# pashtari/factorizer

Measured on AMD Instinct MI355X. Metric: volumes/sec fwd+bwd, Swin Factorizer 128^3, higher is better.
Workload: dtype f32

## Files before the change

factorizer_amd/_native.py:

```python
from __future__ import annotations

import ctypes
import os
import threading

import torch

_HERE = os.path.dirname(os.path.abspath(__file__))
LIB_PATH = os.environ.get("FZ_LIB_PATH") or os.path.join(_HERE, "libfactorizer_hip.so")

FZ_OK = 0
FZ_E_UNSUPPORTED = -2
ABI_VERSION = 7
SOLVER_ID = {"mu": 0, "hals": 1, "cd": 2, "smu": 3}
STORE_F32, STORE_BF16 = 0, 1
PRODUCTS_DEFAULT, PRODUCTS_SPLIT_BF16, PRODUCTS_FP32_MFMA = 0, 1, 2
_products = threading.local()


def products() -> int:
    return getattr(_products, "value", PRODUCTS_DEFAULT)


class use_products:
# ... 150 lines not shown


class BlockPrologue(_c.Structure):
    _fields_ = [("ln_g", _vp), ("ln_b", _vp), ("ln_eps", _f), ("w", _vp), ("t", _vp), ("stats", _vp)]


class GemmDwDesc(_c.Structure):
    _fields_ = [("g", _vp), ("q", _vp), ("w", _vp), ("ln", _i), ("stats", _vp), ("ln_g", _vp), ("ln_b", _vp), ("gadd", _vp),
                ("y", _vp), ("gln", _vp), ("wpart", _vp), ("gw", _vp), ("gb", _vp), ("B", _i), ("C", _i), ("V", _i64),
                ("act_dtype", _i), ("ldgw", _i), ("ldw", _i), ("drop_m", _vp), ("drop_s", _f)]


class WgradDesc(_c.Structure):
    _fields_ = [("p", _vp), ("M", _i), ("pmul", _vp), ("pmul_kind", _i), ("q", _vp * 4), ("nsrc", _i),
                ("src_mode", _i), ("c0", _i), ("Cin", _i), ("K", _i), ("Vq", _i64), ("D", _i), ("H", _i),
                ("W", _i), ("N", _i64), ("Ho", _i), ("Wo", _i), ("stats", _vp), ("qact", _i), ("ln_g", _vp),
                ("ln_b", _vp), ("gw", _vp), ("gbias", _vp), ("accumulate", _i), ("B", _i), ("loader", _i),
                ("act_dtype", _i), ("products", _i)]


_SIGS.update({
    "fz_gcorr_supported": ([_i] * 5, _i),
    "fz_gcorr": ([_vp] * 5 + [_i] * 11 + [_f, _vp], _i),
    "fz_gcorr_wgrad_workspace_bytes": ([_i] * 10, _i64),
    "fz_gcorr_wgrad": ([_vp] * 4 + [_i] * 11 + [_vp], _i),
    "fz_gnmf_supported": ([_i, _i64, _i, _i, _i], _i),
    "fz_gnmf_workspace_bytes": ([_i64, _i, _i64, _i, _i, _i], _i64),
    "fz_gnmf_launches": ([_i, _i, _i], _i),
    "fz_gnmf_fwd": ([_vp] * 6 + [_i64, _i, _i64, _i, _i, _i, _f, _vp, _vp], _i),
    "fz_gnmf_bwd": ([_vp] * 7 + [_i64, _i, _i64, _i, _i, _i, _i, _f, _vp, _vp], _i),
    "fz_nmf_cf_supported": ([_i] * 11, _i),
    "fz_nmf_cf_fwd": ([_vp] * 4 + [_i] * 5 + [_c.POINTER(_i)] + [_i] * 5 + [_f, _i, _vp], _i),
    "fz_nmf_cf_bwd": ([_vp] * 5 + [_i] * 5 + [_c.POINTER(_i)] + [_i] * 7 + [_f, _i, _vp], _i),
    "fz_nmf_pcf_supported": ([_i] * 11, _i),
    "fz_nmf_pcf_fwd": ([_vp] * 4 + [_i] * 8 + [_c.POINTER(_i)] + [_i] * 5 + [_f, _i, _vp], _i),
    "fz_nmf_pcf_bwd": ([_vp] * 5 + [_i] * 8 + [_c.POINTER(_i)] + [_i] * 7 + [_f, _i, _vp], _i),
    "fz_nmf_pcf_bwd_prefers_separate": ([_i] * 4, _i),
    "fz_act_add": ([_vp, _vp, _i64, _i, _vp], _i),
    "fz_mlp_pre_supported": ([_i, _i, _i64, _i], _i),
    "fz_mlp_drop_supported": ([_i, _i, _i64, _i], _i),
    "fz_mlp_chain_drop": ([_c.POINTER(MlpDesc), _c.POINTER(MlpDropout), _vp], _i),
    "fz_conv3_prologue_supported": ([_i] * 4, _i),
    "fz_conv3_fwd2": ([_vp] * 4 + [_i] * 8 + [_c.POINTER(BlockPrologue), _vp], _i),
    "fz_upcat2": ([_vp, _vp, _vp, _i, _vp, _vp, _vp] + [_i] * 7 + [_c.POINTER(BlockPrologue), _vp], _i),
    "fz_gemm": ([_c.POINTER(GemmDesc), _vp], _i),
    "fz_gemm_bx_enable": ([_i], _i),
    "fz_gemm_lnbwd_partials": ([_c.POINTER(GemmDesc)], _i64),
    "fz_reduce_rows": ([_vp, _i64, _i, _vp, _vp, _vp], _i),
    "fz_adamw_step": ([_vp, _vp, _vp, _vp, _i64, _f, _f, _f, _f, _f, _i, _f, _vp], _i),
    "fz_sw_gather": ([_vp, _vp] + [_i] * 10 + [_vp], _i),
    "fz_sw_accumulate": ([_vp] * 6 + [_f] + [_i] * 10 + [_vp], _i),
    "fz_sw_finalize": ([_vp, _vp, _i, _i64, _vp], _i),
    "fz_sw_gather2": ([_vp, _vp] + [_i] * 11 + [_vp], _i),
    "fz_sw_accumulate2": ([_vp] * 6 + [_f] + [_i] * 11 + [_vp], _i),
    "fz_sw_finalize2": ([_vp, _vp, _vp, _i, _i64, _i, _vp], _i),
    "fz_mlp_supported": ([_i, _i, _i64], _i),
    "fz_mlp_partials": ([_i, _i64], _i64),
    "fz_mlp_wgrad_rows": ([_i, _i64], _i),
    "fz_gemm_dw_rows": ([_i, _i64], _i),
    "fz_gemm_dw_workspace_bytes": ([_i, _i64], _i64),
    "fz_gemm_dw": ([_c.POINTER(GemmDwDesc), _vp], _i),
    "fz_mlp_wgrad_workspace_bytes": ([_i, _i64], _i64),
    "fz_mlp_chain": ([_c.POINTER(MlpDesc), _vp], _i),
    "fz_head_bwd_rows": ([], _i),
    "fz_head_bwd_workspace_bytes": ([], _i64),
    "fz_head_bwd": ([_vp, _vp, _vp, _vp, _vp, _i, _i, _i, _i64, _i, _vp], _i),
# ... 47 lines not shown
```

factorizer_amd/csrc/nmf_cf.h:

```cpp
#pragma once
#include <cstdlib>

#include "fz_common.h"
#include "nmf_core.h"
#include "nmf_gram.h"

namespace fz {

struct CfGeom {
  int B, C, D, H, W;
  int h;
  int G0, G1, G2;
  int s0, s1, s2;
  int accumulate;
  int divisor;
  float gscale_div;
  int64_t plane;
};

struct CfWave {
  using F = float;
  int lane;
  __device__ __forceinline__ int col(int j) const {
    const int jp = j >> 2, e = j & 3;
    return (((jp * 4 + (lane >> 4)) * 8 + ((lane >> 1) & 7)) * 8) + (lane & 1) * 4 + e;
  }
  __device__ __forceinline__ float sum(float v) const { return wave_sum(v); }
  __device__ __forceinline__ void sum8(float (&v)[8]) const { wave_sum8(v, lane); }
  __device__ __forceinline__ void st_priv(float* base, int idx, float v) const { base[idx * 64 + lane] = v; }
  __device__ __forceinline__ float ld_priv(const float* base, int idx) const { return base[idx * 64 + lane]; }
  __device__ __forceinline__ void st_uni(float* base, int idx, float v) const {
    if (lane == 0) base[idx] = v;
  }
  __device__ __forceinline__ float ld_uni(const float* base, int idx) const { return base[idx]; }
  __device__ __forceinline__ float ld_uni_global(const float* p, int idx) const { return p[idx]; }
  __device__ __forceinline__ float ld_v0(const float* v0, int j, int r, int R) const { return v0[col(j) * R + r]; }
  __device__ __forceinline__ float keep_col(int, float v) const { return v; }
  __device__ __forceinline__ void fence() const { __builtin_amdgcn_fence(__ATOMIC_ACQ_REL, "wavefront"); }
  static constexpr bool kDistRows = true;
  __device__ __forceinline__ float sum8_dist(const float (&v)[8]) const { return wave_sum8_dist(v, lane); }
  __device__ __forceinline__ float grp_take(float d, int m) const {
    return __int_as_float(__builtin_amdgcn_readlane(__float_as_int(d), 8 * m));
  }
  __device__ __forceinline__ bool grp_below(int n) const { return (lane >> 3) < n; }
  __device__ __forceinline__ void st_grp(float* base, int i0, int stride, float d) const {
    if ((lane & 7) == 0) base[i0 + (lane >> 3) * stride] = d;
  }
  __device__ __forceinline__ float ld_grp_global(const float* p, int i0, int stride) const { return p[i0 + (lane >> 3) * stride]; }
  __device__ __forceinline__ float ld_grp(const float* base, int i0, int stride) const { return base[i0 + (lane >> 3) * stride]; }
  __device__ __forceinline__ float grp_sum(float d) const { return wave_group_sum(d); }
  __device__ __forceinline__ float mask_rows(float d, int mreal) const { return (lane >> 3) < mreal ? d : 0.f; }
// ... 143 lines not shown
    aload<2>(cf_at(p, o), a);
    aload<2>(cf_at(p, o2), b);
    return make_float4(a[0], a[1], b[0], b[1]);
  }
  return ld4(cf_at(p, o));
}
template <bool HALF, typename AT>
__device__ __forceinline__ void cf_st4(AT* p, unsigned o, unsigned o2, float4 v) {
  if (HALF) {
    const float a[2] = {v.x, v.y}, b[2] = {v.z, v.w};
    astore<2>(cf_at(p, o), a);
    astore<2>(cf_at(p, o2), b);
  } else {
    st4(cf_at(p, o), v);
  }
}

struct CfTileId { int b, hh, g0, g1, gq; };

template <int WPB>
__device__ __forceinline__ CfTileId cf_tile_id(const CfGeom& q, int64_t blk) {
  const unsigned ngrp = (unsigned)(q.G2 / WPB);
  unsigned t = (unsigned)blk;
  CfTileId id;
  id.gq = (int)(t % ngrp); t /= ngrp;
  id.g1 = (int)(t % (unsigned)q.G1); t /= (unsigned)q.G1;
  id.g0 = (int)(t % (unsigned)q.G0); t /= (unsigned)q.G0;
  id.hh = (int)(t % (unsigned)q.h);
  id.b = (int)(t / (unsigned)q.h);
  return id;
}

template <int WPB>
__device__ __forceinline__ void cf_tile_decode(const CfGeom& q, const CfTileId& id, int tid, int64_t& base, int64_t& V,
                                               unsigned (&off)[2], int (&lidx)[2], unsigned (&off2)[2]) {
  using TL = CfTile<WPB>;
  V = q.plane;
  base = ((int64_t)id.b * q.C + (int64_t)id.hh * 8) * V;
#pragma unroll
  for (int k = 0; k < 2; ++k) {
    const int idx = tid + k * TL::NT;
    const int row = idx / TL::CHUNKS, chunk = idx % TL::CHUNKS;
    int z0 = id.g0 * 8 + (row >> 3) - q.s0; if (z0 < 0) z0 += q.D;
    int z1 = id.g1 * 8 + (row & 7) - q.s1; if (z1 < 0) z1 += q.H;
    int z2 = id.gq * WPB * 8 + chunk * 4 - q.s2; if (z2 < 0) z2 += q.W;
    off[k] = (unsigned)((z0 * q.H + z1) * q.W + z2);
    int z2b = z2 + 2; if (z2b >= q.W) z2b -= q.W;
    off2[k] = (unsigned)((z0 * q.H + z1) * q.W + z2b);
    lidx[k] = TL::at(row, chunk);
  }
}

template <int WPB>
__device__ __forceinline__ int cf_owner_lidx(int lane, int wave, int jp) {
  return CfTile<WPB>::at((jp * 4 + (lane >> 4)) * 8 + ((lane >> 1) & 7), wave * 2 + (lane & 1));
}

template <int WPB>
__device__ __forceinline__ void cf_to_owner(float* S, const int (&lidx)[2], int own0, int own1, float (&x)[8][8]) {
  using TL = CfTile<WPB>;
#pragma unroll
  for (int s = 0; s < 4; ++s) {
#pragma unroll
    for (int c = 0; c < 2; ++c)
#pragma unroll
      for (int k = 0; k < 2; ++k)
        *reinterpret_cast<float4*>(S + c * 64 * TL::LW + lidx[k]) =
            make_float4(x[2 * s + c][k * 4 + 0], x[2 * s + c][k * 4 + 1], x[2 * s + c][k * 4 + 2], x[2 * s + c][k * 4 + 3]);
    __syncthreads();
#pragma unroll
    for (int c = 0; c < 2; ++c) {
      const float4 a0 = *reinterpret_cast<const float4*>(S + c * 64 * TL::LW + own0);
      const float4 a1 = *reinterpret_cast<const float4*>(S + c * 64 * TL::LW + own1);
      x[2 * s + c][0] = a0.x; x[2 * s + c][1] = a0.y; x[2 * s + c][2] = a0.z; x[2 * s + c][3] = a0.w;
      x[2 * s + c][4] = a1.x; x[2 * s + c][5] = a1.y; x[2 * s + c][6] = a1.z; x[2 * s + c][7] = a1.w;
    }
    __syncthreads();
  }
}


template <typename AT>
int cf_bwd_gram_launch(const AT* t, const float* v0, const AT* ga, AT* gt, const CfGeom& q, int64_t nmat, int T, int G,
// ... 4 lines not shown
```

factorizer_amd/csrc/nmf_cf.hip:

```cpp
#include "nmf_cf.h"

namespace fz {

template <int R, int SOLVER, int WPB, bool HALF, typename AT>
__device__ __forceinline__ void cf_fwd_tile_body(const AT* __restrict__ t, const float* __restrict__ u0,
                                                 const float* __restrict__ v0, AT* __restrict__ out, const CfGeom& q,
                                                 const CfTileId& id, int T, float eps, float* S) {
  using TL = CfTile<WPB>;
  const int tid = threadIdx.x, lane = tid & 63, wave = tid >> 6;
  int64_t base, V;
  unsigned off[2], off2[2];
  int lidx[2];
  cf_tile_decode<WPB>(q, id, tid, base, V, off, lidx, off2);
  const int own0 = cf_owner_lidx<WPB>(lane, wave, 0), own1 = cf_owner_lidx<WPB>(lane, wave, 1);

  float x[8][8];
#pragma unroll
  for (int dd = 0; dd < 8; ++dd)
#pragma unroll
    for (int k = 0; k < 2; ++k) {
      const float4 v = cf_ld4<HALF>(t + base + dd * V, off[k], off2[k]);
      x[dd][k * 4 + 0] = v.x; x[dd][k * 4 + 1] = v.y; x[dd][k * 4 + 2] = v.z; x[dd][k * 4 + 3] = v.w;
    }
  cf_to_owner<WPB>(S, lidx, own0, own1, x);

  CfWave w{lane};
  float u[8][R], v[8][R];
  nmf_forward_wave<8, 8, R, SOLVER>(w, u0, v0, x, u, v, 8, T, eps);

  const float dv = (float)q.divisor;
  const bool dv_pow2 = cf_pow2(dv);
  asm volatile("" : "+s"(base));
  float4 old[8][2];
  if (q.accumulate) {
#pragma unroll
    for (int dd = 0; dd < 8; ++dd)
#pragma unroll
      for (int k = 0; k < 2; ++k) old[dd][k] = cf_ld4<HALF>(out + base + dd * V, off[k], off2[k]);
  }
#pragma unroll
  for (int s = 0; s < 4; ++s) {
#pragma unroll
    for (int c = 0; c < 2; ++c) {
      *reinterpret_cast<float4*>(S + c * 64 * TL::LW + own0) =
          make_float4(x[2 * s + c][0], x[2 * s + c][1], x[2 * s + c][2], x[2 * s + c][3]);
      *reinterpret_cast<float4*>(S + c * 64 * TL::LW + own1) =
          make_float4(x[2 * s + c][4], x[2 * s + c][5], x[2 * s + c][6], x[2 * s + c][7]);
    }
    __syncthreads();
#pragma unroll
    for (int c = 0; c < 2; ++c)
#pragma unroll
      for (int k = 0; k < 2; ++k) {
        const float4 z = *reinterpret_cast<const float4*>(S + c * 64 * TL::LW + lidx[k]);
        float4 o;
        if (q.accumulate) {
          o = old[2 * s + c][k];
          o.x += z.x; o.y += z.y; o.z += z.z; o.w += z.w;
        } else {
          o = make_float4(0.0f + z.x, 0.0f + z.y, 0.0f + z.z, 0.0f + z.w);
        }
        if (q.divisor > 1) o = cf_divide4(o, dv, dv_pow2);
        cf_st4<HALF>(out + base + (2 * s + c) * V, off[k], off2[k], o);
      }
    __syncthreads();
  }
}

template <int R, int SOLVER, int WPB, bool HALF, typename AT>
__global__ __launch_bounds__(WPB * 64, (WPB == 8 || R >= 2) ? 2 : 4) void nmf_cf_fwd_tile_kernel(const AT* __restrict__ t,
                                                                   const float* __restrict__ u0,
                                                                   const float* __restrict__ v0,
                                                                   AT* __restrict__ out, CfGeom q, int T, float eps,
                                                                   int xcd_remap) {
  extern __shared__ __attribute__((aligned(16))) float fz_lds_tile[];
  cf_fwd_tile_body<R, SOLVER, WPB, HALF, AT>(t, u0, v0, out, q, cf_tile_id<WPB>(q, cf_logical_block(xcd_remap)), T, eps, fz_lds_tile);
}

template <int R, int SOLVER, typename AT>
__global__ __launch_bounds__(256, (R == 1 && (SOLVER == SOLVER_HALS || SOLVER == SOLVER_CD)) ? 2 : 1) void nmf_cf_bwd_kernel(const AT* __restrict__ t, const float* __restrict__ u0,
                                                            const float* __restrict__ v0,
                                                            const AT* __restrict__ ga, AT* __restrict__ gt,
                                                            CfGeom q, int64_t nmat, int T, int G, float eps,
                                                            int relu_gate, int xcd_remap) {
  extern __shared__ __attribute__((aligned(16))) float fz_lds_cf[];
  const int lane = threadIdx.x & 63, wave = threadIdx.x >> 6;
  const int64_t mat = cf_logical_block(xcd_remap) * (blockDim.x >> 6) + wave;
  if (mat >= nmat) return;
  CfWave w{lane};
  CfAddr a;
  cf_decode(q, mat, lane, a);
  Hist<8, 8, R> h;
  h.carve(fz_lds_cf + wave * Hist<8, 8, R>::floats(G), G);
  float x[8][8], g[8][8];
  cf_load(t, a, x);
  cf_load(ga, a, g);
  cf_divide(g, q.gscale_div);
  nmf_backward_wave<8, 8, R, SOLVER>(w, u0, v0, x, g, h, 8, T, G, eps, nullptr, nullptr);
#pragma unroll
  for (int dd = 0; dd < 8; ++dd)
#pragma unroll
    for (int jp = 0; jp < 2; ++jp) {
      AT* p = gt + a.base + dd * a.V + a.off[jp];
      float r[4];
#pragma unroll
      for (int e = 0; e < 4; ++e) {
        const float gv = g[dd][jp * 4 + e];
        r[e] = (!relu_gate || x[dd][jp * 4 + e] > 0.f) ? gv : 0.f;
      }
// ... 73 lines not shown
        if (q.accumulate) {
          const float4 o = old[2 * s + c][k];
          z.x += o.x; z.y += o.y; z.z += o.z; z.w += o.w;
        }
        cf_st4<HALF>(gt + base + (2 * s + c) * V, off[k], off2[k], z);
      }
    __syncthreads();
  }
}

template <int R, int SOLVER, int WPB, bool HALF, typename AT>
__global__ __launch_bounds__(WPB * 64, (R == 1 && (SOLVER == SOLVER_HALS || SOLVER == SOLVER_CD) && (WPB == 4 || WPB == 1)) ? 2 : 1) void nmf_cf_bwd_tile_kernel(
    const AT* __restrict__ t, const float* __restrict__ u0, const float* __restrict__ v0,
    const AT* __restrict__ ga, AT* __restrict__ gt, CfGeom q, int T, int G, float eps, int relu_gate,
    int xcd_remap) {
  extern __shared__ __attribute__((aligned(16))) float fz_lds_cf[];
  cf_bwd_tile_body<R, SOLVER, WPB, HALF, AT>(t, u0, v0, ga, gt, q, cf_tile_id<WPB>(q, cf_logical_block(xcd_remap)), T, G, eps,
                                             relu_gate, fz_lds_cf);
}


static int cf_geom(CfGeom& q, int B, int C, int D, int H, int W, const int* shift, int accumulate, int divisor) {
  if (B < 0 || C < 8 || (C % 8) || D < 8 || H < 8 || W < 8 || (D % 8) || (H % 8) || (W % 8))
    return fail(FZ_E_SHAPE, "fz_nmf_cf: needs C % 8 == 0 and spatial dims multiples of 8");
  if (!shift) return fail(FZ_E_ARG, "fz_nmf_cf: shift is null");
  if ((int64_t)D * H * W >= ((int64_t)1 << 30)) return fail(FZ_E_UNSUPPORTED, "fz_nmf_cf: 2^30 or more voxels per channel plane");
  q.B = B; q.C = C; q.D = D; q.H = H; q.W = W; q.h = C / 8; q.G0 = D / 8; q.G1 = H / 8; q.G2 = W / 8;
  int s[3];
  const int S[3] = {D, H, W};
  for (int i = 0; i < 3; ++i) { s[i] = shift[i] % S[i]; if (s[i] < 0) s[i] += S[i]; }
  if (s[2] % 2) return fail(FZ_E_UNSUPPORTED, "fz_nmf_cf: W-axis shift must be even");
  q.s0 = s[0]; q.s1 = s[1]; q.s2 = s[2];
  q.accumulate = accumulate; q.divisor = divisor; q.gscale_div = 1.0f;
  q.plane = (int64_t)D * H * W;
#ifdef FZ_PROBE_PLANE_PAD
  q.plane += FZ_PROBE_PLANE_PAD;
#endif
  return FZ_OK;
}

}

using namespace fz;

extern "C" int fz_nmf_cf_supported(int C, int D, int H, int W, int d, int pd, int ph, int pw, int R, int T, int Tgrad) {
  if (d != 8 || pd != 8 || ph != 8 || pw != 8 || (C % 8) || (D % 8) || (H % 8) || (W % 8)) return 0;
  if (R < 1 || R > 2 || T < 0 || (int64_t)D * H * W >= ((int64_t)1 << 30)) return 0;
  const int G = Tgrad < 0 ? 0 : (Tgrad > T ? T : Tgrad);
  const int per_wave = ((G + 1) * R * 8 * 64 + (G + 1) * 8 * R + G * (8 * R + R * R)) * 4;
  return per_wave <= 160 * 1024 ? 1 : 0;
}

template <typename AT>
static int cf_fwd_launch(const AT* t, const float* u0, const float* v0, AT* out, int B, int C, int D,
                         int H, int W, const int* shift, int accumulate, int divisor, int R, int T,
                         int solver, float eps, fz_stream_t stream) {
  CfGeom q;
  int rc = cf_geom(q, B, C, D, H, W, shift, accumulate, divisor);
  if (rc != FZ_OK) return rc;
  if (!t || !u0 || !v0 || !out) return fail(FZ_E_ARG, "fz_nmf_cf_fwd: null pointer");
  if (R < 1 || R > 2) return fail(FZ_E_UNSUPPORTED, "fz_nmf_cf_fwd: rank 1..2");
  if (solver < FZ_SOLVER_MU || solver > FZ_SOLVER_SMU) return fail(FZ_E_ARG, "fz_nmf_cf_fwd: bad solver");
  if (B == 0) return FZ_OK;
  const int64_t nmat = (int64_t)B * q.h * q.G0 * q.G1 * q.G2;
  if (nmat >= (int64_t)1 << 31) return fail(FZ_E_UNSUPPORTED, "fz_nmf_cf: more than 2^31 matrices");
  int wpb = 16;
  if (wpb > q.G2) wpb = q.G2;
  if (wpb < 1) wpb = 1;
  const int xr = 1 | (tile_order() << 1);
  hipStream_t st = (hipStream_t)stream;
  const int tile = FZ_KNOB("FZ_CF_TILE").set ? FZ_KNOB("FZ_CF_TILE").val : 1;
  const bool half = (q.s2 % 4) != 0;
  if (half || (tile && (q.G2 % 8) == 0)) {
    const int twpb = (q.G2 % 8) == 0 ? 8 : ((q.G2 % 4) == 0 ? 4 : 1);
    const unsigned nblk = (unsigned)(nmat / twpb);
#define FZ_CF_TILE(RR, SS, WW, HH)                                                                          \
  do {                                                                                                      \
    auto kern = nmf_cf_fwd_tile_kernel<RR, SS, WW, HH, AT>;                                                   \
    const int lds = CfTile<WW>::STAGE_FLOATS * (int)sizeof(float);                                          \
    hipLaunchKernelGGL(kern, dim3(nblk), dim3(64 * WW), lds, st, t, u0, v0, out, q, T, eps, xr);            \
  } while (0)
#define FZ_CF_TILE_W(RR, SS)                                                                                \
  do {                                                                                                      \
    if (half) { if (twpb == 8) FZ_CF_TILE(RR, SS, 8, true); else if (twpb == 4) FZ_CF_TILE(RR, SS, 4, true); else FZ_CF_TILE(RR, SS, 1, true); } \
    else FZ_CF_TILE(RR, SS, 8, false);                                                                      \
  } while (0)
    if (R == 1) { FZ_SOLVER_CASES(FZ_CF_TILE_W, 1); }
    else { FZ_SOLVER_CASES(FZ_CF_TILE_W, 2); }
    FZ_LAUNCH_CHECK();
    return FZ_OK;
  }
  dim3 grid((unsigned)((nmat + wpb - 1) / wpb)), block(64 * wpb);
#define FZ_CF_FWD(RR, SS) hipLaunchKernelGGL((nmf_cf_fwd_kernel<RR, SS, AT>), grid, block, 0, st, t, u0, v0, out, q, nmat, T, eps, xr)
  if (R == 1) { FZ_SOLVER_CASES(FZ_CF_FWD, 1); }
  else { FZ_SOLVER_CASES(FZ_CF_FWD, 2); }
  FZ_LAUNCH_CHECK();
  return FZ_OK;
}

extern "C" int fz_nmf_cf_fwd(const void* t, const float* u0, const float* v0, void* out, int B, int C, int D,
                             int H, int W, const int* shift, int accumulate, int divisor, int R, int T,
                             int solver, float eps, int act_dtype, fz_stream_t stream) {
  if (act_dtype == FZ_STORE_F32)
    return cf_fwd_launch<float>((const float*)t, u0, v0, (float*)out, B, C, D, H, W, shift, accumulate, divisor, R, T,
                                solver, eps, stream);
  if (act_dtype == FZ_STORE_BF16)
    return cf_fwd_launch<bf16>((const bf16*)t, u0, v0, (bf16*)out, B, C, D, H, W, shift, accumulate, divisor, R, T,
                               solver, eps, stream);
  return fail(FZ_E_ARG, "fz_nmf_cf_fwd: bad act_dtype");
}

template <typename AT>
static int cf_bwd_launch(const AT* t, const float* u0, const float* v0, const AT* ga, AT* gt, int B,
                         int C, int D, int H, int W, const int* shift, int accumulate, int nshift,
                         int relu_gate, int R, int T, int Tgrad, int solver, float eps, fz_stream_t stream) {
  CfGeom q;
  int rc = cf_geom(q, B, C, D, H, W, shift, accumulate, 1);
  if (rc != FZ_OK) return rc;
  if (!t || !u0 || !v0 || !ga || !gt) return fail(FZ_E_ARG, "fz_nmf_cf_bwd: null pointer");
  if (R < 1 || R > 2) return fail(FZ_E_UNSUPPORTED, "fz_nmf_cf_bwd: rank 1..2");
  if (solver < FZ_SOLVER_MU || solver > FZ_SOLVER_SMU) return fail(FZ_E_ARG, "fz_nmf_cf_bwd: bad solver");
  if (B == 0) return FZ_OK;
  q.gscale_div = (float)(nshift > 1 ? nshift : 1);
  const int G = Tgrad < 0 ? 0 : (Tgrad > T ? T : Tgrad);
  const int64_t nmat = (int64_t)B * q.h * q.G0 * q.G1 * q.G2;
  if (nmat >= (int64_t)1 << 31) return fail(FZ_E_UNSUPPORTED, "fz_nmf_cf: more than 2^31 matrices");
  const int per_wave = (R == 1 ? Hist<8, 8, 1>::floats(G) : Hist<8, 8, 2>::floats(G)) * (int)sizeof(float);
  if (per_wave > 160 * 1024) return fail(FZ_E_UNSUPPORTED, "fz_nmf_cf_bwd: history exceeds LDS");
  int wpb = 65536 / per_wave;
  if (wpb > 4) wpb = 4;
  if (wpb > 8) wpb = 8;
  if (wpb < 1) wpb = 1;
  const int xr = 1 | (tile_order() << 1);
  hipStream_t st = (hipStream_t)stream;
  const int tile = FZ_KNOB("FZ_CF_TILE_BWD").set ? FZ_KNOB("FZ_CF_TILE_BWD").val : 1;
  const bool half = (q.s2 % 4) != 0;
  if (half || (tile && (q.G2 % 4) == 0)) {
    const int twpb = (q.G2 % 4) == 0 ? 4 : 1;
    const bool gram_on = !(FZ_KNOB("FZ_CF_GRAM").set && FZ_KNOB("FZ_CF_GRAM").val == 0);
    const bool gram_wins = !(sizeof(AT) == 4 && accumulate && nmat >= 32768);
    if (gram_on && gram_wins && R == 1 && solver == FZ_SOLVER_HALS && relu_gate && G >= 1) {
      rc = cf_bwd_gram_launch<AT>(t, v0, ga, gt, q, nmat, T, G, eps, xr, st);
// ... 55 lines not shown
```

factorizer_amd/functional.py:

```python
from __future__ import annotations

import math
import os

import torch

from . import _native as N


def _dev_guard(t: torch.Tensor):
    return torch.cuda.device(t.device)


class KernelTimer:

    def __init__(self, only=None):
        self.records = []
        self.only = None if only is None else set(only)

    def launch(self, name, nbytes, fn, cols=0, flops=0):
        if self.only is not None and name not in self.only:
            return fn()
        s = torch.cuda.Event(enable_timing=True)
        e = torch.cuda.Event(enable_timing=True)
# ... 26 lines not shown

def _timed(name, nbytes, fn, cols=0, flops=0):
    if _timer is None:
        return fn()
    return _timer.launch(name, nbytes, fn, cols, flops)


class Geometry:

    def __init__(self, channels, spatial, head_dim, patch, shifts):
        self.C = int(channels)
        self.spatial = tuple(int(s) for s in spatial)
        self.d = int(head_dim)
        self.patch = tuple(int(p) for p in patch)
        self.shifts = [tuple(int(v) for v in s) for s in shifts]
        if self.C % self.d:
            raise ValueError(f"channels {self.C} not divisible by head_dim {self.d}")
        for s, p in zip(self.spatial, self.patch):
            if s % p:
                raise ValueError(f"spatial size {self.spatial} not divisible by patch size {self.patch}")
        self.h = self.C // self.d
        self.grid = tuple(s // p for s, p in zip(self.spatial, self.patch))
        self.G = math.prod(self.grid)
        self.P = math.prod(self.patch)
        self.nshift = len(self.shifts)
        nd = len(self.spatial)
        if nd > 3:
            raise ValueError("at most 3 spatial dims")
        pad = 3 - nd
        self.s3 = (1,) * pad + self.spatial
        self.p3 = (1,) * pad + self.patch
        self.shifts3 = [(0,) * pad + s for s in self.shifts]
        self._carr = N.shifts_array(self.shifts3)

    def y_shape(self, B):
        return (self.nshift * B * self.h, self.G, self.d, self.P)


def _swm_fwd_raw(x, geo: Geometry, relu=False, div=1):
    B = x.shape[0]
    y = torch.empty(geo.y_shape(B), dtype=x.dtype, device=x.device)
    if x.dtype == torch.float32:
        es = 4
    elif x.dtype in (torch.bfloat16, torch.float16):
        es = 2
        if x.dtype == torch.float16 and (relu or div > 1):
            raise TypeError("SWMatricize with fused arithmetic: float32 or bfloat16 (float16 only moves bits)")
    else:
        raise TypeError(f"SWMatricize: unsupported dtype {x.dtype}")
    with _dev_guard(x):
        rc = _timed("swm_fwd", (1 + geo.nshift) * x.numel() * es, lambda: N.lib().fz_swm_fwd(
            x.data_ptr(), y.data_ptr(), B, geo.C, *geo.s3, geo.d, *geo.p3, geo.nshift, geo._carr, es,
            int(relu), int(div), N.stream_ptr(x)))
    N.check(rc, "fz_swm_fwd")
    return y


def _swm_inv_raw(y, geo: Geometry, average=True, gate=None):
    ad = N.act_dtype(y)
    if gate is not None and gate.dtype != y.dtype:
        raise TypeError("SWMatricize.inverse_forward: gate and y must have the same dtype")
    B = y.shape[0] // (geo.nshift * geo.h)
    x = torch.empty((B, geo.C, *geo.spatial), dtype=y.dtype, device=y.device)
    with _dev_guard(y):
        rc = _timed("swm_inv", (1 + geo.nshift) * x.numel() * y.element_size(), lambda: N.lib().fz_swm_inv(
            y.data_ptr(), x.data_ptr(), B, geo.C, *geo.s3, geo.d, *geo.p3, geo.nshift, geo._carr,
# ... 201 lines not shown
class GNMFDecomposeFn(torch.autograd.Function):
    @staticmethod
    def forward(ctx, x, u0, v0, T, G, solver, eps):
        x, u0, v0 = x.contiguous(), u0.contiguous(), v0.contiguous()
        _, u, v = _gnmf_fwd_raw(x, u0, v0, T, solver, eps, want_uv=True)
        ctx.save_for_backward(x, u0, v0)
        ctx.cfg = (T, G, solver, eps)
        return u, v

    @staticmethod
    def backward(ctx, gu, gv):
        x, u0, v0 = ctx.saved_tensors
        T, G, solver, eps = ctx.cfg
        if G <= 0:
            return torch.zeros_like(x), None, None, None, None, None, None
        gx = _gnmf_bwd_raw(x, u0, v0, None, gu.contiguous(), gv.contiguous(), T, G, solver, eps)
        return gx, None, None, None, None, None, None


def gnmf(x, u0, v0, T, G, solver, eps=1e-16):
    return GNMFFn.apply(x, u0, v0, T, G, solver, eps)


def gnmf_decompose(x, u0, v0, T, G, solver, eps=1e-16):
    return GNMFDecomposeFn.apply(x, u0, v0, T, G, solver, eps)


def nmf_cf_supported(geo: Geometry, R, T, G) -> bool:
    if len(geo.spatial) != 3 or any(s[2] % 2 for s in geo.shifts):
        return False
    return bool(N.lib().fz_nmf_cf_supported(geo.C, *geo.spatial, geo.d, *geo.patch, int(R), int(T), int(G)))


def nmf_pcf_supported(geo: Geometry, R, T, G) -> bool:
    if os.environ.get("FZ_NMF_PCF", "1") == "0":
        return False
    return bool(N.lib().fz_nmf_pcf_supported(geo.C, *geo.s3, geo.d, *geo.p3, int(R), int(T), int(G)))


def nmf_core_supported(geo: Geometry, R, T, G) -> bool:
    return nmf_cf_supported(geo, R, T, G) or nmf_pcf_supported(geo, R, T, G)


class FactCoreFn(torch.autograd.Function):

    @staticmethod
    def forward(ctx, t, u0, v0, geo, T, G, solver, eps, relu_gate):
        t = t.contiguous()
        u0, v0 = u0.contiguous(), v0.contiguous()
        B = t.shape[0]
        out = torch.empty_like(t)
        R = u0.shape[1]
        es = t.element_size()
        nb = 2 * es * t.numel()
        ad = N.act_dtype(t)
        hot = nmf_cf_supported(geo, R, T, G)
        with _dev_guard(t):
            for w, s in enumerate(geo.shifts3):
                arr = (N._i * 3)(*s)
                last = geo.nshift if w == geo.nshift - 1 else 1
                N.set_tile_order(w & 1)
                if hot:
                    rc = _timed(f"nmf_cf_fwd_{geo.C}x" + "x".join(str(v) for v in geo.spatial), nb + (es * t.numel() if w else 0), cols=t.numel() // geo.C, fn=lambda: N.lib().fz_nmf_cf_fwd(
                        t.data_ptr(), u0.data_ptr(), v0.data_ptr(), out.data_ptr(), B, geo.C, *geo.spatial, arr,
                        int(w > 0), last, R, T, N.SOLVER_ID[solver], eps, ad, N.stream_ptr(t)))
                else:
                    rc = _timed(f"nmf_pcf_fwd_{geo.C}x" + "x".join(str(v) for v in geo.spatial), nb + (es * t.numel() if w else 0), cols=t.numel() // geo.C, fn=lambda: N.lib().fz_nmf_pcf_fwd(
                        t.data_ptr(), u0.data_ptr(), v0.data_ptr(), out.data_ptr(), B, geo.C, *geo.s3, *geo.p3, arr,
                        int(w > 0), last, R, T, N.SOLVER_ID[solver], eps, ad, N.stream_ptr(t)))
                N.check(rc, "fz_nmf_cf_fwd" if hot else "fz_nmf_pcf_fwd")
            N.set_tile_order(0)
        ctx.save_for_backward(t, u0, v0)
        ctx.cfg = (geo, T, G, solver, eps, relu_gate)
        return out

    @staticmethod
    def backward(ctx, ga):
        t, u0, v0 = ctx.saved_tensors
        geo, T, G, solver, eps, relu_gate = ctx.cfg
        if G <= 0:
            return (torch.zeros_like(t),) + (None,) * 8
        ga = ga.contiguous()
        if ga.dtype != t.dtype:
            ga = ga.to(t.dtype)
        gt = torch.empty_like(t)
        B = t.shape[0]
        R = u0.shape[1]
        es = t.element_size()
        nb = 3 * es * t.numel()
        ad = N.act_dtype(t)
        hot = nmf_cf_supported(geo, R, T, G)
        with _dev_guard(t):
            for w, s in enumerate(geo.shifts3):
                arr = (N._i * 3)(*s)
                N.set_tile_order(w & 1)
                if hot:
                    rc = _timed(f"nmf_cf_bwd_{geo.C}x" + "x".join(str(v) for v in geo.spatial), nb + (es * t.numel() if w else 0), cols=t.numel() // geo.C, fn=lambda: N.lib().fz_nmf_cf_bwd(
                        t.data_ptr(), u0.data_ptr(), v0.data_ptr(), ga.data_ptr(), gt.data_ptr(), B, geo.C,
                        *geo.spatial, arr, int(w > 0), geo.nshift, int(relu_gate), R, T, G, N.SOLVER_ID[solver], eps,
                        ad, N.stream_ptr(t)))
                elif w > 0 and N.lib().fz_nmf_pcf_bwd_prefers_separate(*geo.p3, ad):
                    tmp = torch.empty_like(gt)
                    rc = _timed(f"nmf_pcf_bwd_{geo.C}x" + "x".join(str(v) for v in geo.spatial), nb, cols=t.numel() // geo.C, fn=lambda: N.lib().fz_nmf_pcf_bwd(
# ... 255 lines not shown
```

include/factorizer_hip.h:

```cpp
#ifndef FACTORIZER_HIP_H
#define FACTORIZER_HIP_H

#include <stdint.h>

#ifdef __cplusplus
extern "C" {
#endif

#define FZ_OK 0
#define FZ_E_SHAPE (-1)
#define FZ_E_UNSUPPORTED (-2)
#define FZ_E_HIP (-3)
#define FZ_E_ARG (-4)

#define FZ_STORE_F32 0
#define FZ_STORE_BF16 1

#define FZ_SOLVER_MU 0
#define FZ_SOLVER_HALS 1
#define FZ_SOLVER_CD 2
#define FZ_SOLVER_SMU 3

typedef void* fz_stream_t;

// ... 14 lines not shown

int fz_swm_inv(const void* y, void* x, int B, int C, int D, int H, int W, int d, int pd,
               int ph, int pw, int nshift, const int* shifts, int average, const void* gate,
               int act_dtype, fz_stream_t stream);

int fz_nmf_fwd(const void* x, const float* u0, const float* v0, void* y, float* u_out,
               float* v_out, int64_t nmat, int M, int N, int R, int T, int solver, float eps,
               int act_dtype, fz_stream_t stream);

int fz_nmf_bwd(const void* x, const float* u0, const float* v0, const void* gy,
               const float* gu, const float* gv, void* gx, int64_t nmat, int M, int N, int R,
               int T, int Tgrad, int solver, float eps, int act_dtype, fz_stream_t stream);

int fz_nmf_supported(int M, int N, int R, int T, int Tgrad);

int fz_gnmf_supported(int M, int64_t N, int R, int T, int Tgrad);
int64_t fz_gnmf_workspace_bytes(int64_t nmat, int M, int64_t N, int R, int T, int backward);
int fz_gnmf_launches(int T, int Tgrad, int backward);
int fz_gnmf_fwd(const float* x, const float* u0, const float* v0, float* y, float* u_out, float* v_out,
                int64_t nmat, int M, int64_t N, int R, int T, int solver, float eps, void* workspace,
                fz_stream_t stream);
int fz_gnmf_bwd(const float* x, const float* u0, const float* v0, const float* gy, const float* gu,
                const float* gv, float* gx, int64_t nmat, int M, int64_t N, int R, int T, int Tgrad, int solver,
                float eps, void* workspace, fz_stream_t stream);

int fz_nmf_cf_supported(int C, int D, int H, int W, int d, int pd, int ph, int pw, int R, int T, int Tgrad);
int fz_nmf_cf_fwd(const void* t, const float* u0, const float* v0, void* out, int B, int C, int D,
                  int H, int W, const int* shift, int accumulate, int divisor, int R, int T,
                  int solver, float eps, int act_dtype, fz_stream_t stream);
int fz_nmf_cf_bwd(const void* t, const float* u0, const float* v0, const void* ga, void* gt, int B,
                  int C, int D, int H, int W, const int* shift, int accumulate, int nshift,
                  int relu_gate, int R, int T, int Tgrad, int solver, float eps, int act_dtype,
                  fz_stream_t stream);

int fz_nmf_pcf_supported(int C, int D, int H, int W, int d, int pd, int ph, int pw, int R, int T, int Tgrad);
int fz_nmf_pcf_fwd(const void* t, const float* u0, const float* v0, void* out, int B, int C, int D, int H, int W,
                   int pd, int ph, int pw, const int* shift, int accumulate, int divisor, int R, int T, int solver,
                   float eps, int act_dtype, fz_stream_t stream);
int fz_nmf_pcf_bwd(const void* t, const float* u0, const float* v0, const void* ga, void* gt, int B, int C, int D,
                   int H, int W, int pd, int ph, int pw, const int* shift, int accumulate, int nshift, int relu_gate,
                   int R, int T, int Tgrad, int solver, float eps, int act_dtype, fz_stream_t stream);
int fz_nmf_pcf_bwd_prefers_separate(int pd, int ph, int pw, int act_dtype);
int fz_act_add(void* dst, const void* src, int64_t n, int act_dtype, fz_stream_t stream);

#define FZ_LOAD_PLAIN 0
#define FZ_LOAD_S2D 1
#define FZ_LOAD_K3 2
#define FZ_EPI_PLAIN 0
#define FZ_EPI_D2S 1
#define FZ_EPI_LNBWD 2
#define FZ_LOAD_S2D_2D 3
#define FZ_LOAD_K3_2D 4
#define FZ_EPI_D2S_2D 3
#define FZ_ACT_NONE 0
#define FZ_ACT_RELU 1
#define FZ_ACT_GELU 2

#define FZ_PRODUCTS_DEFAULT 0
#define FZ_PRODUCTS_SPLIT_BF16 1
#define FZ_PRODUCTS_FP32_MFMA 2

typedef struct fz_gemm_desc {
  const void* x[4];
  int nsrc;
  int src_mode;
  int c0;
// ... 274 lines not shown
```

Before: 127.9.

## Store rank-1 NMF factors from first shift window and rebuild output in second pass

Result: faster. 130.2, median of 6 (+1.8%).

```diff
diff --git a/factorizer_amd/_native.py b/factorizer_amd/_native.py
--- a/factorizer_amd/_native.py
+++ b/factorizer_amd/_native.py
@@ -206,6 +206,9 @@
     "fz_nmf_cf_supported": ([_i] * 11, _i),
     "fz_nmf_cf_fwd": ([_vp] * 4 + [_i] * 5 + [_c.POINTER(_i)] + [_i] * 5 + [_f, _i, _vp], _i),
     "fz_nmf_cf_bwd": ([_vp] * 5 + [_i] * 5 + [_c.POINTER(_i)] + [_i] * 7 + [_f, _i, _vp], _i),
+    "fz_nmf_cf_factors_supported": ([_i] * 12 + [_c.POINTER(_i)], _i),
+    "fz_nmf_cf_fwd_store_factors": ([_vp] * 5 + [_i] * 5 + [_c.POINTER(_i)] + [_i] * 3 + [_f, _i, _vp], _i),
+    "fz_nmf_cf_fwd_from_factors": ([_vp] * 6 + [_i] * 5 + [_c.POINTER(_i)] * 2 + [_i] * 4 + [_f, _i, _vp], _i),
     "fz_nmf_pcf_supported": ([_i] * 11, _i),
     "fz_nmf_pcf_fwd": ([_vp] * 4 + [_i] * 8 + [_c.POINTER(_i)] + [_i] * 5 + [_f, _i, _vp], _i),
     "fz_nmf_pcf_bwd": ([_vp] * 5 + [_i] * 8 + [_c.POINTER(_i)] + [_i] * 7 + [_f, _i, _vp], _i),
diff --git a/factorizer_amd/csrc/nmf_cf.h b/factorizer_amd/csrc/nmf_cf.h
--- a/factorizer_amd/csrc/nmf_cf.h
+++ b/factorizer_amd/csrc/nmf_cf.h
@@ -16,7 +16,10 @@
   int divisor;
   float gscale_div;
   int64_t plane;
+  int ps0, ps1, ps2;
 };
+
+enum { CF_PLAIN = 0, CF_STORE_FACTORS = 1, CF_FROM_FACTORS = 2 };
 
 struct CfWave {
   using F = float;
@@ -226,6 +229,17 @@
 }
 
 template <int WPB>
+__device__ __forceinline__ void cf_chunk_voxel(const CfGeom& q, const CfTileId& id, int tid, int k, int& row, int& chunk,
+                                               int& z0, int& z1, int& z2) {
+  using TL = CfTile<WPB>;
+  const int idx = tid + k * TL::NT;
+  row = idx / TL::CHUNKS; chunk = idx % TL::CHUNKS;
+  z0 = id.g0 * 8 + (row >> 3) - q.s0; if (z0 < 0) z0 += q.D;
+  z1 = id.g1 * 8 + (row & 7) - q.s1; if (z1 < 0) z1 += q.H;
+  z2 = id.gq * WPB * 8 + chunk * 4 - q.s2; if (z2 < 0) z2 += q.W;
+}
+
+template <int WPB>
 __device__ __forceinline__ void cf_tile_decode(const CfGeom& q, const CfTileId& id, int tid, int64_t& base, int64_t& V,
                                                unsigned (&off)[2], int (&lidx)[2], unsigned (&off2)[2]) {
   using TL = CfTile<WPB>;
@@ -233,16 +247,35 @@
   base = ((int64_t)id.b * q.C + (int64_t)id.hh * 8) * V;
 #pragma unroll
   for (int k = 0; k < 2; ++k) {
-    const int idx = tid + k * TL::NT;
-    const int row = idx / TL::CHUNKS, chunk = idx % TL::CHUNKS;
-    int z0 = id.g0 * 8 + (row >> 3) - q.s0; if (z0 < 0) z0 += q.D;
-    int z1 = id.g1 * 8 + (row & 7) - q.s1; if (z1 < 0) z1 += q.H;
-    int z2 = id.gq * WPB * 8 + chunk * 4 - q.s2; if (z2 < 0) z2 += q.W;
+    int row, chunk, z0, z1, z2;
+    cf_chunk_voxel<WPB>(q, id, tid, k, row, chunk, z0, z1, z2);
     off[k] = (unsigned)((z0 * q.H + z1) * q.W + z2);
     int z2b = z2 + 2; if (z2b >= q.W) z2b -= q.W;
     off2[k] = (unsigned)((z0 * q.H + z1) * q.W + z2b);
     lidx[k] = TL::at(row, chunk);
   }
+}
+
+template <int WPB>
+__device__ __forceinline__ unsigned cf_prev_patch(const CfGeom& q, const CfTileId& id, int tid, int k) {
+  int row, chunk, z0, z1, z2;
+  cf_chunk_voxel<WPB>(q, id, tid, k, row, chunk, z0, z1, z2);
+  z0 += q.ps0; if (z0 >= q.D) z0 -= q.D;
+  z1 += q.ps1; if (z1 >= q.H) z1 -= q.H;
+  z2 += q.ps2; if (z2 >= q.W) z2 -= q.W;
+  return (unsigned)(((z0 >> 3) * q.G1 + (z1 >> 3)) * q.G2 + (z2 >> 3));
+}
+
+template <typename AT>
+__device__ __forceinline__ float4 cf_first_window(float u, const float4& v) {
+  float p0 = u * v.x, p1 = u * v.y, p2 = u * v.z, p3 = u * v.w;
+  asm("" : "+v"(p0), "+v"(p1), "+v"(p2), "+v"(p3));
+  const f32v4 f = {0.0f + p0, 0.0f + p1, 0.0f + p2, 0.0f + p3};
+  if constexpr (sizeof(AT) == 2) {
+    const f32v4 r = __builtin_convertvector(__builtin_convertvector(f, bf16v4), f32v4);
+    return make_float4(r[0], r[1], r[2], r[3]);
+  }
+  return make_float4(f[0], f[1], f[2], f[3]);
 }
 
 template <int WPB>
diff --git a/factorizer_amd/csrc/nmf_cf.hip b/factorizer_amd/csrc/nmf_cf.hip
--- a/factorizer_amd/csrc/nmf_cf.hip
+++ b/factorizer_amd/csrc/nmf_cf.hip
@@ -2,10 +2,11 @@
 
 namespace fz {
 
-template <int R, int SOLVER, int WPB, bool HALF, typename AT>
+template <int R, int SOLVER, int WPB, bool HALF, typename AT, int FORM>
 __device__ __forceinline__ void cf_fwd_tile_body(const AT* __restrict__ t, const float* __restrict__ u0,
-                                                 const float* __restrict__ v0, AT* __restrict__ out, const CfGeom& q,
-                                                 const CfTileId& id, int T, float eps, float* S) {
+                                                 const float* __restrict__ v0, AT* __restrict__ out, float* vfac, float* ufac,
+                                                 const CfGeom& q, const CfTileId& id, int T, float eps, float* S) {
+  static_assert(FORM == CF_PLAIN || (R == 1 && WPB == 8 && !HALF), "the factor forms: rank 1, 8 patches per workgroup, W-axis shifts = 0 (mod 4)");
   using TL = CfTile<WPB>;
   const int tid = threadIdx.x, lane = tid & 63, wave = tid >> 6;
   int64_t base, V;
@@ -28,11 +29,41 @@
   float u[8][R], v[8][R];
   nmf_forward_wave<8, 8, R, SOLVER>(w, u0, v0, x, u, v, 8, T, eps);
 
+  const int64_t bh = (int64_t)id.b * q.h + id.hh;
+  const int64_t vol = (int64_t)q.D * q.H * q.W;
+  if constexpr (FORM == CF_STORE_FACTORS) {
+    *reinterpret_cast<float4*>(S + own0) = make_float4(v[0][0], v[1][0], v[2][0], v[3][0]);
+    *reinterpret_cast<float4*>(S + own1) = make_float4(v[4][0], v[5][0], v[6][0], v[7][0]);
+    __syncthreads();
+    float* vp = vfac + bh * vol;
+#pragma unroll
+    for (int k = 0; k < 2; ++k) st4(cf_at(vp, off[k]), *reinterpret_cast<const float4*>(S + lidx[k]));
+    if (lane == 0) {
+      float* up = ufac + ((((bh * q.G0 + id.g0) * q.G1 + id.g1) * q.G2 + id.gq * WPB + wave) << 3);
+      st4(up, make_float4(u[0][0], u[1][0], u[2][0], u[3][0]));
+      st4(up + 4, make_float4(u[4][0], u[5][0], u[6][0], u[7][0]));
+    }
+    return;
+  }
+
   const float dv = (float)q.divisor;
   const bool dv_pow2 = cf_pow2(dv);
   asm volatile("" : "+s"(base));
   float4 old[8][2];
-  if (q.accumulate) {
+  float4 pv[2];
+  float pu[2][8];
+  if constexpr (FORM == CF_FROM_FACTORS) {
+    const float* vp = vfac + bh * vol;
+    const float* up = ufac + ((bh * q.G0 * q.G1 * q.G2) << 3);
+#pragma unroll
+    for (int k = 0; k < 2; ++k) {
+      pv[k] = ld4(cf_at(vp, off[k]));
+      const float* pk = up + (cf_prev_patch<WPB>(q, id, tid, k) << 3);
+      const float4 a = ld4(pk), b = ld4(pk + 4);
+      pu[k][0] = a.x; pu[k][1] = a.y; pu[k][2] = a.z; pu[k][3] = a.w;
+      pu[k][4] = b.x; pu[k][5] = b.y; pu[k][6] = b.z; pu[k][7] = b.w;
+    }
+  } else if (q.accumulate) {
 #pragma unroll
     for (int dd = 0; dd < 8; ++dd)
 #pragma unroll
@@ -54,7 +85,10 @@
       for (int k = 0; k < 2; ++k) {
         const float4 z = *reinterpret_cast<const float4*>(S + c * 64 * TL::LW + lidx[k]);
         float4 o;
-        if (q.accumulate) {
+        if constexpr (FORM == CF_FROM_FACTORS) {
+          o = cf_first_window<AT>(pu[k][2 * s + c], pv[k]);
+          o.x += z.x; o.y += z.y; o.z += z.z; o.w += z.w;
+        } else if (q.accumulate) {
           o = old[2 * s + c][k];
           o.x += z.x; o.y += z.y; o.z += z.z; o.w += z.w;
         } else {
@@ -67,14 +101,15 @@
   }
 }
 
-template <int R, int SOLVER, int WPB, bool HALF, typename AT>
+template <int R, int SOLVER, int WPB, bool HALF, typename AT, int FORM>
 __global__ __launch_bounds__(WPB * 64, (WPB == 8 || R >= 2) ? 2 : 4) void nmf_cf_fwd_tile_kernel(const AT* __restrict__ t,
                                                                    const float* __restrict__ u0,
                                                                    const float* __restrict__ v0,
-                                                                   AT* __restrict__ out, CfGeom q, int T, float eps,
-                                                                   int xcd_remap) {
+                                                                   AT* __restrict__ out, float* vfac, float* ufac,
+                                                                   CfGeom q, int T, float eps, int xcd_remap) {
   extern __shared__ __attribute__((aligned(16))) float fz_lds_tile[];
-  cf_fwd_tile_body<R, SOLVER, WPB, HALF, AT>(t, u0, v0, out, q, cf_tile_id<WPB>(q, cf_logical_block(xcd_remap)), T, eps, fz_lds_tile);
+  cf_fwd_tile_body<R, SOLVER, WPB, HALF, AT, FORM>(t, u0, v0, out, vfac, ufac, q, cf_tile_id<WPB>(q, cf_logical_block(xcd_remap)), T, eps,
+                                                   fz_lds_tile);
 }
 
 template <int R, int SOLVER, typename AT>
@@ -214,6 +249,7 @@
   if (s[2] % 2) return fail(FZ_E_UNSUPPORTED, "fz_nmf_cf: W-axis shift must be even");
   q.s0 = s[0]; q.s1 = s[1]; q.s2 = s[2];
   q.accumulate = accumulate; q.divisor = divisor; q.gscale_div = 1.0f;
+  q.ps0 = q.ps1 = q.ps2 = 0;
   q.plane = (int64_t)D * H * W;
 #ifdef FZ_PROBE_PLANE_PAD
   q.plane += FZ_PROBE_PLANE_PAD;
@@ -258,9 +294,9 @@
     const unsigned nblk = (unsigned)(nmat / twpb);
 #define FZ_CF_TILE(RR, SS, WW, HH)                                                                          \
   do {                                                                                                      \
-    auto kern = nmf_cf_fwd_tile_kernel<RR, SS, WW, HH, AT>;                                                   \
+    auto kern = nmf_cf_fwd_tile_kernel<RR, SS, WW, HH, AT, CF_PLAIN>;                                         \
     const int lds = CfTile<WW>::STAGE_FLOATS * (int)sizeof(float);                                          \
-    hipLaunchKernelGGL(kern, dim3(nblk), dim3(64 * WW), lds, st, t, u0, v0, out, q, T, eps, xr);            \
+    hipLaunchKernelGGL(kern, dim3(nblk), dim3(64 * WW), lds, st, t, u0, v0, out, (float*)nullptr, (float*)nullptr, q, T, eps, xr); \
   } while (0)
 #define FZ_CF_TILE_W(RR, SS)                                                                                \
   do {                                                                                                      \
@@ -290,6 +326,85 @@
     return cf_fwd_launch<bf16>((const bf16*)t, u0, v0, (bf16*)out, B, C, D, H, W, shift, accumulate, divisor, R, T,
                                solver, eps, stream);
   return fail(FZ_E_ARG, "fz_nmf_cf_fwd: bad act_dtype");
+}
+
+static void cf_norm_shift(const int* shift, int D, int H, int W, int (&s)[3]) {
+  const int S[3] = {D, H, W};
+  for (int i = 0; i < 3; ++i) { s[i] = shift[i] % S[i]; if (s[i] < 0) s[i] += S[i]; }
+}
+
+extern "C" int fz_nmf_cf_factors_supported(int C, int D, int H, int W, int d, int pd, int ph, int pw, int R, int T, int Tgrad,
+                                           int nshift, const int* shifts) {
+  if (!fz_nmf_cf_supported(C, D, H, W, d, pd, ph, pw, R, T, Tgrad)) return 0;
+  if (R != 1 || nshift != 2 || !shifts || (W % 64)) return 0;
+  for (int w = 0; w < 2; ++w) {
+    int s[3];
+    cf_norm_shift(shifts + 3 * w, D, H, W, s);
+    if (s[2] % 4) return 0;
+  }
+  return 1;
+}
+
+template <typename AT>
+static int cf_fwd_factors_launch(const AT* t, const float* u0, const float* v0, AT* out, float* vfac, float* ufac, int B, int C,
+                                 int D, int H, int W, const int* shift, const int* prev_shift, int form, int divisor, int R, int T,
+                                 int solver, float eps, fz_stream_t stream, const char* who) {
+  CfGeom q;
+  int rc = cf_geom(q, B, C, D, H, W, shift, form == CF_FROM_FACTORS, divisor);
+  if (rc != FZ_OK) return rc;
+  if (!t || !u0 || !v0 || !vfac || !ufac || (form == CF_FROM_FACTORS && (!out || !prev_shift))) return fail(FZ_E_ARG, who);
+  if (R != 1) return fail(FZ_E_UNSUPPORTED, "fz_nmf_cf_fwd factor forms: rank 1 only");
+  if (W % 64) return fail(FZ_E_UNSUPPORTED, "fz_nmf_cf_fwd factor forms: W must be a multiple of 64");
+  if (solver < FZ_SOLVER_MU || solver > FZ_SOLVER_SMU) return fail(FZ_E_ARG, "fz_nmf_cf_fwd factor forms: bad solver");
+  if (divisor < 1) return fail(FZ_E_ARG, "fz_nmf_cf_fwd factor forms: divisor < 1");
+  if (q.s2 % 4) return fail(FZ_E_UNSUPPORTED, "fz_nmf_cf_fwd factor forms: W-axis shift must be a multiple of 4");
+  if (form == CF_FROM_FACTORS) {
+    int ps[3];
+    cf_norm_shift(prev_shift, D, H, W, ps);
+    if (ps[2] % 4) return fail(FZ_E_UNSUPPORTED, "fz_nmf_cf_fwd factor forms: W-axis shift must be a multiple of 4");
+    q.ps0 = ps[0]; q.ps1 = ps[1]; q.ps2 = ps[2];
+  }
+  if (B == 0) return FZ_OK;
+  const int64_t nmat = (int64_t)B * q.h * q.G0 * q.G1 * q.G2;
+  if (nmat >= (int64_t)1 << 31) return fail(FZ_E_UNSUPPORTED, "fz_nmf_cf: more than 2^31 matrices");
+  const int xr = 1 | (tile_order() << 1);
+  hipStream_t st = (hipStream_t)stream;
+  const unsigned nblk = (unsigned)(nmat / 8);
+  const int lds = CfTile<8>::STAGE_FLOATS * (int)sizeof(float);
+#define FZ_CF_FACT(FF, SS)                                                                                          \
+  hipLaunchKernelGGL((nmf_cf_fwd_tile_kernel<1, SS, 8, false, AT, FF>), dim3(nblk), dim3(512), lds, st, t, u0, v0, out, vfac, \
+                     ufac, q, T, eps, xr)
+  if (form == CF_STORE_FACTORS) { FZ_SOLVER_CASES(FZ_CF_FACT, CF_STORE_FACTORS); }
+  else { FZ_SOLVER_CASES(FZ_CF_FACT, CF_FROM_FACTORS); }
+  FZ_LAUNCH_CHECK();
+  return FZ_OK;
+}
+
+extern "C" int fz_nmf_cf_fwd_store_factors(const void* t, const float* u0, const float* v0, float* vfac, float* ufac, int B,
+                                           int C, int D, int H, int W, const int* shift, int R, int T, int solver, float eps,
+                                           int act_dtype, fz_stream_t stream) {
+  const char* who = "fz_nmf_cf_fwd_store_factors: null pointer (t, u0, v0, vfac or ufac)";
+  if (act_dtype == FZ_STORE_F32)
+    return cf_fwd_factors_launch<float>((const float*)t, u0, v0, nullptr, vfac, ufac, B, C, D, H, W, shift, nullptr,
+                                        CF_STORE_FACTORS, 1, R, T, solver, eps, stream, who);
+  if (act_dtype == FZ_STORE_BF16)
+    return cf_fwd_factors_launch<bf16>((const bf16*)t, u0, v0, nullptr, vfac, ufac, B, C, D, H, W, shift, nullptr,
+                                       CF_STORE_FACTORS, 1, R, T, solver, eps, stream, who);
+  return fail(FZ_E_ARG, "fz_nmf_cf_fwd_store_factors: bad act_dtype");
+}
+
+extern "C" int fz_nmf_cf_fwd_from_factors(const void* t, const float* u0, const float* v0, const float* vfac,
+                                          const float* ufac, void* out, int B, int C, int D, int H, int W, const int* shift,
+                                          const int* prev_shift, int divisor, int R, int T, int solver, float eps, int act_dtype,
+                                          fz_stream_t stream) {
+  const char* who = "fz_nmf_cf_fwd_from_factors: null pointer (t, u0, v0, vfac, ufac, out or prev_shift)";
+  if (act_dtype == FZ_STORE_F32)
+    return cf_fwd_factors_launch<float>((const float*)t, u0, v0, (float*)out, const_cast<float*>(vfac), const_cast<float*>(ufac),
+                                        B, C, D, H, W, shift, prev_shift, CF_FROM_FACTORS, divisor, R, T, solver, eps, stream, who);
+  if (act_dtype == FZ_STORE_BF16)
+    return cf_fwd_factors_launch<bf16>((const bf16*)t, u0, v0, (bf16*)out, const_cast<float*>(vfac), const_cast<float*>(ufac),
+                                       B, C, D, H, W, shift, prev_shift, CF_FROM_FACTORS, divisor, R, T, solver, eps, stream, who);
+  return fail(FZ_E_ARG, "fz_nmf_cf_fwd_from_factors: bad act_dtype");
 }
 
 template <typename AT>
diff --git a/factorizer_amd/functional.py b/factorizer_amd/functional.py
--- a/factorizer_amd/functional.py
+++ b/factorizer_amd/functional.py
@@ -82,6 +82,7 @@
         self.p3 = (1,) * pad + self.patch
         self.shifts3 = [(0,) * pad + s for s in self.shifts]
         self._carr = N.shifts_array(self.shifts3)
+        self._factors_ok = {}
 
     def y_shape(self, B):
         return (self.nshift * B * self.h, self.G, self.d, self.P)
@@ -349,6 +350,17 @@
     return bool(N.lib().fz_nmf_cf_supported(geo.C, *geo.spatial, geo.d, *geo.patch, int(R), int(T), int(G)))
 
 
+def nmf_cf_factors_supported(geo: Geometry, R, T, G) -> bool:
+    if len(geo.spatial) != 3:
+        return False
+    k = (int(R), int(T), int(G))
+    ok = geo._factors_ok.get(k)
+    if ok is None:
+        ok = geo._factors_ok[k] = bool(N.lib().fz_nmf_cf_factors_supported(geo.C, *geo.spatial, geo.d, *geo.patch, *k,
+                                                                          geo.nshift, geo._carr))
+    return ok
+
+
 def nmf_pcf_supported(geo: Geometry, R, T, G) -> bool:
     if os.environ.get("FZ_NMF_PCF", "1") == "0":
         return False
@@ -372,20 +384,38 @@
         nb = 2 * es * t.numel()
         ad = N.act_dtype(t)
         hot = nmf_cf_supported(geo, R, T, G)
+        key = ("nmf_cf_fwd_" if hot else "nmf_pcf_fwd_") + f"{geo.C}x" + "x".join(str(v) for v in geo.spatial)
+        st = N.stream_ptr(t)
         with _dev_guard(t):
-            for w, s in enumerate(geo.shifts3):
-                arr = (N._i * 3)(*s)
-                last = geo.nshift if w == geo.nshift - 1 else 1
-                N.set_tile_order(w & 1)
-                if hot:
-                    rc = _timed(f"nmf_cf_fwd_{geo.C}x" + "x".join(str(v) for v in geo.spatial), nb + (es * t.numel() if w else 0), cols=t.numel() // geo.C, fn=lambda: N.lib().fz_nmf_cf_fwd(
-                        t.data_ptr(), u0.data_ptr(), v0.data_ptr(), out.data_ptr(), B, geo.C, *geo.spatial, arr,
-                        int(w > 0), last, R, T, N.SOLVER_ID[solver], eps, ad, N.stream_ptr(t)))
-                else:
-                    rc = _timed(f"nmf_pcf_fwd_{geo.C}x" + "x".join(str(v) for v in geo.spatial), nb + (es * t.numel() if w else 0), cols=t.numel() // geo.C, fn=lambda: N.lib().fz_nmf_pcf_fwd(
-                        t.data_ptr(), u0.data_ptr(), v0.data_ptr(), out.data_ptr(), B, geo.C, *geo.s3, *geo.p3, arr,
-                        int(w > 0), last, R, T, N.SOLVER_ID[solver], eps, ad, N.stream_ptr(t)))
-                N.check(rc, "fz_nmf_cf_fwd" if hot else "fz_nmf_pcf_fwd")
+            if hot and nmf_cf_factors_supported(geo, R, T, G):
+                vfac = torch.empty((B, geo.h, *geo.spatial), device=t.device, dtype=torch.float32)
+                ufac = torch.empty((B * geo.h * geo.G, 8), device=t.device, dtype=torch.float32)
+                s0, s1 = ((N._i * 3)(*s) for s in geo.shifts3)
+                nf = 4 * (t.numel() // 8)
+                N.set_tile_order(0)
+                rc = _timed(key, es * t.numel() + nf, cols=t.numel() // geo.C, fn=lambda: N.lib().fz_nmf_cf_fwd_store_factors(
+                    t.data_ptr(), u0.data_ptr(), v0.data_ptr(), vfac.data_ptr(), ufac.data_ptr(), B, geo.C, *geo.spatial, s0,
+                    R, T, N.SOLVER_ID[solver], eps, ad, st))
+                N.check(rc, "fz_nmf_cf_fwd_store_factors")
+                N.set_tile_order(1)
+                rc = _timed(key, 2 * es * t.numel() + nf, cols=t.numel() // geo.C, fn=lambda: N.lib().fz_nmf_cf_fwd_from_factors(
+                    t.data_ptr(), u0.data_ptr(), v0.data_ptr(), vfac.data_ptr(), ufac.data_ptr(), out.data_ptr(), B, geo.C,
+                    *geo.spatial, s1, s0, 2, R, T, N.SOLVER_ID[solver], eps, ad, st))
+                N.check(rc, "fz_nmf_cf_fwd_from_factors")
+            else:
+                for w, s in enumerate(geo.shifts3):
+                    arr = (N._i * 3)(*s)
+                    last = geo.nshift if w == geo.nshift - 1 else 1
+                    N.set_tile_order(w & 1)
+                    if hot:
+                        rc = _timed(key, nb + (es * t.numel() if w else 0), cols=t.numel() // geo.C, fn=lambda: N.lib().fz_nmf_cf_fwd(
+                            t.data_ptr(), u0.data_ptr(), v0.data_ptr(), out.data_ptr(), B, geo.C, *geo.spatial, arr,
+                            int(w > 0), last, R, T, N.SOLVER_ID[solver], eps, ad, st))
+                    else:
+                        rc = _timed(key, nb + (es * t.numel() if w else 0), cols=t.numel() // geo.C, fn=lambda: N.lib().fz_nmf_pcf_fwd(
+                            t.data_ptr(), u0.data_ptr(), v0.data_ptr(), out.data_ptr(), B, geo.C, *geo.s3, *geo.p3, arr,
+                            int(w > 0), last, R, T, N.SOLVER_ID[solver], eps, ad, st))
+                    N.check(rc, "fz_nmf_cf_fwd" if hot else "fz_nmf_pcf_fwd")
             N.set_tile_order(0)
         ctx.save_for_backward(t, u0, v0)
         ctx.cfg = (geo, T, G, solver, eps, relu_gate)
diff --git a/include/factorizer_hip.h b/include/factorizer_hip.h
--- a/include/factorizer_hip.h
+++ b/include/factorizer_hip.h
@@ -70,6 +70,15 @@
                   int C, int D, int H, int W, const int* shift, int accumulate, int nshift,
                   int relu_gate, int R, int T, int Tgrad, int solver, float eps, int act_dtype,
                   fz_stream_t stream);
+
+int fz_nmf_cf_factors_supported(int C, int D, int H, int W, int d, int pd, int ph, int pw, int R, int T, int Tgrad,
+                                int nshift, const int* shifts);
+int fz_nmf_cf_fwd_store_factors(const void* t, const float* u0, const float* v0, float* vfac, float* ufac, int B,
+                                int C, int D, int H, int W, const int* shift, int R, int T, int solver, float eps,
+                                int act_dtype, fz_stream_t stream);
+int fz_nmf_cf_fwd_from_factors(const void* t, const float* u0, const float* v0, const float* vfac, const float* ufac,
+                               void* out, int B, int C, int D, int H, int W, const int* shift, const int* prev_shift,
+                               int divisor, int R, int T, int solver, float eps, int act_dtype, fz_stream_t stream);
 
 int fz_nmf_pcf_supported(int C, int D, int H, int W, int d, int pd, int ph, int pw, int R, int T, int Tgrad);
 int fz_nmf_pcf_fwd(const void* t, const float* u0, const float* v0, void* out, int B, int C, int D, int H, int W,
```
